# maxall41/RustSASA

Measured on AMD Instinct MI355X. Metric: structures/sec on AF2 E. coli proteome (100 pts, 1.4 A probe), higher is better.
Workload: dtype f32

## Files before the change

rustsasa_amd/csrc/context.cpp:

```cpp
#include "engine_internal.h"

namespace rsasa {

const char *tuning_env(const char *name)
{
    static const bool on = [] { const char *v = std::getenv("RSASA_TUNING"); return v && std::atoi(v) != 0; }();
    return on ? std::getenv(name) : nullptr;
}

void generate_sphere_points(size_t n, float *x, float *y, float *z)
{
    const float pi = 3.14159274101257324219f;
    const float angle_increment = (2.0f * pi) * 1.618034f;
    const float inv_n = 1.0f / (float)n;
    for (size_t i = 0; i < n; i++) {
        const float fi = (float)i;
        const float t = fi * inv_n;
        const float inclination = acosf(1.0f - 2.0f * t);
        const float azimuth = angle_increment * fi;
        const float si = sinf(inclination);
        x[i] = si * cosf(azimuth);
        y[i] = si * sinf(azimuth);
        z[i] = cosf(inclination);
    }
// ... 410 lines not shown
        RS_HIP(ctx, hs.h_segments.regrow((n_seg_all + n_seg_all / 2 + 64) * sizeof(Segment)));
    }
    Segment *h_segments = static_cast<Segment *>(hs.h_segments.p);
    write_segments(bt.structure_offsets_host, S, h_segments, reinterpret_cast<uint32_t *>(h_segments + n_seg));

    const bool has_id = bt.id != nullptr;
    if ((rc = W.reserve_grid(ctx, N, S, n_seg_all, ctx->cell_capacity, has_tail, has_id))) return rc;
    if ((rc = W.reserve_occlusion(ctx, lat, N, has_id, has_id, !bt.out_atom_sasa))) return rc;
    const bool keep_ids = W.keep_ids;
    if (keep_ids && pd.id32) return fail(ctx, RSASA_ERR_INTERNAL, "folded ids on a batch the per-atom kernels take");

    if (n_seg_all)
        RS_HIP(ctx, hipMemcpyAsync(W.segments.p, h_segments, n_seg_all * sizeof(Segment),
                                   hipMemcpyHostToDevice, st));

    BatchView v{};
    v.x = bt.x; v.y = bt.y; v.z = bt.z; v.radius = bt.radius; v.id = bt.id;
    v.id32 = pd.id32;
    v.ids_check = (has_id && !pd.ids_needed_known && !keep_ids && !tuning_env("RSASA_NO_ID_CHECK")) ? 1u : 0u;
    hs.ids_check = v.ids_check != 0u;
    v.large_sids = reinterpret_cast<const uint32_t *>((const Segment *)W.segments.p + n_seg);
    v.n_large = (uint32_t)n_large;
    v.ids_tables = ctx->ids_unordered_hint ? 1u : 0u;
    v.radius8 = pd.radius8;
    v.radius_table = pd.radius_table;
    v.residue_offsets = bt.residue_offsets;
    v.n_atoms = (uint32_t)N; v.n_structures = (uint32_t)S; v.n_residues = (uint32_t)R;
    v.n_segments = (uint32_t)n_seg;
    v.probe = pd.probe;
    v.atom_sasa = bt.out_atom_sasa;
    W.grid_view(v);
    W.occlusion_view(v);
    v.residue_sasa = (R && bt.residue_offsets) ? bt.out_residue_sasa : nullptr;
    v.neighbor_counts = bt.out_neighbor_counts;

    if (ctx->timing) RS_HIP(ctx, hipEventRecord(W.ev[0], st));
    launch_grid_prepare(v, st);
    rsasa_context::Workspace &other = ctx->ws[pd.ws ^ 1];
    const bool chain = other.occ_recorded && !tuning_env("RSASA_FREE_OVERLAP");
    const bool overlap = ctx->overlap_tail && has_tail;
    if (overlap && (rc = ensure_side_stream(ctx))) return rc;
    if (overlap) {
        launch_sort_lds(v, st);
        RS_HIP(ctx, hipEventRecord(ctx->ev_fork, st));
        RS_HIP(ctx, hipStreamWaitEvent(ctx->side_stream, ctx->ev_fork, 0));
        launch_sort_tail(v, ctx->side_stream);
// ... 176 lines not shown
    if (e == hipSuccess) e = new_stream(ctx, &ctx->stream.h, 2);
    for (int w = 0; w < rsasa_context::kInFlight; w++) {
        for (int i = 0; i < 5 && e == hipSuccess; i++) e = hipEventCreate(&ctx->ws[w].ev[i].h);
        if (e == hipSuccess) e = hipEventCreateWithFlags(&ctx->ws[w].ev_occ.h, hipEventDisableTiming);
    }
    if (e == hipSuccess) e = hipEventCreateWithFlags(&ctx->ev_fork.h, hipEventDisableTiming);
    if (e == hipSuccess) e = hipEventCreateWithFlags(&ctx->ev_join.h, hipEventDisableTiming);
    if (e == hipSuccess) e = hipEventCreateWithFlags(&ctx->ev_link.h, hipEventDisableTiming);
    for (int i = 0; i < rsasa_context::kSlots && e == hipSuccess; i++) e = hipEventCreateWithFlags(&ctx->ev_copy[i].h, hipEventDisableTiming);
    for (int i = 0; i < rsasa_context::kSlots && e == hipSuccess; i++) e = hipEventCreateWithFlags(&ctx->ev_d2h[i].h, hipEventDisableTiming);
    for (int i = 0; i < rsasa_context::kSlots && e == hipSuccess; i++) {
        e = ctx->slot[i].h_status.regrow(sizeof(BatchStatus));
        if (e == hipSuccess) std::memset(ctx->slot[i].h_status.p, 0, sizeof(BatchStatus));
        if (e == hipSuccess) e = hipEventCreateWithFlags(&ctx->ev_done[i].h, hipEventDisableTiming);
    }
    if (e != hipSuccess) {
        rsasa_context_destroy(ctx);
        return RSASA_ERR_HIP;
    }
    if (const char *v = tuning_env("RSASA_OCCLUSION_KERNEL")) ctx->tuning.kernel_version = std::atoi(v);
    if (const char *v = tuning_env("RSASA_ATOMS_PER_WAVE")) ctx->tuning.atoms_per_wave = (uint32_t)std::atoi(v);
    if (const char *v = tuning_env("RSASA_OVERLAP_TAIL")) ctx->overlap_tail = std::atoi(v) != 0;
    if (const char *v = tuning_env("RSASA_SMALL_PATH")) ctx->small_path = std::atoi(v) != 0;
    *out_ctx = ctx;
    return RSASA_OK;
}

extern "C" {

int rsasa_context_destroy(rsasa_context_t *ctx)
{
    if (!ctx) return RSASA_OK;
    if (HostStream *hs = ctx->host_stream) {
        {
            std::unique_lock<std::mutex> lk(hs->mu);
            hs->cv_done.wait(lk, [&] { for (auto &j : hs->jobs) if (!j->done) return false; return true; });
            hs->quit = true;
        }
        hs->cv_work.notify_all();
        for (auto &t : hs->th)
            if (t.joinable()) t.join();
        for (rsasa_context *sc : hs->sub) rsasa_context_destroy(sc);
        delete hs;
        ctx->host_stream = nullptr;
    }
    DeviceGuard guard(ctx->device);
// ... 253 lines not shown
```

rustsasa_amd/csrc/device_types.h:

```cpp
#pragma once
#include <hip/hip_runtime.h>
#include <stdint.h>

namespace rsasa {

struct StructGrid {
    float min_x, min_y, min_z;
    float inv_cell;
    uint32_t dim_x, dim_y, dim_z;
    uint32_t cell_base;
    float max_r;
    float cell_size;
    uint32_t n_cells;
    uint32_t atom_begin;
    uint32_t n_atoms;
    uint32_t sorted_base;
    uint32_t in_lds;
    uint32_t odd_radii;
};
static_assert(sizeof(StructGrid) == 64, "StructGrid layout");

struct StructAcc {
    int min_x, min_y, min_z;
    int max_x, max_y, max_z;
// ... 63 lines not shown
    StructGrid *grids;
    uint32_t *sid_sorted;
    uint32_t *cell_of, *rank_of;
    uint32_t *deferred_list;
    uint32_t *claim;
    uint32_t *ids_seg;
    uint32_t ids_seg_words;
    uint32_t *cells;
    uint64_t cell_capacity;
    uint4 *windows;
    uint32_t window_capacity;
    uint32_t *scan_block_sums;
    GridSums *grid_sums;
    float4 *sorted_xyzr;
    uint32_t *sorted_orig;
    uint64_t *sorted_id;
    uint32_t *sorted_id32;
    BatchStatus *status;
    float *atom_sasa;
    float *residue_sasa;
    uint32_t *neighbor_counts;
    uint32_t *defer_flag;
    float max_r_override = __builtin_nanf("");
};

struct NbInfo {
    unsigned long long total;
    unsigned long long max_k;
    unsigned long long spill_entries;
    unsigned long long spill_atoms;
    unsigned long long spill_cursor;
    unsigned long long spill_recs;
    unsigned long long mismatch;
    unsigned long long pad;
};
static_assert(sizeof(NbInfo) == 64, "NbInfo layout");
struct NbKey {
    unsigned long long key;
    float thr;
    uint32_t pad;
};
struct NbSpillRec {
    unsigned long long off, base;
    uint32_t k, pad;
};
struct NbArgs {
// ... 71 lines not shown
void launch_accessible_points(const PtArgs &a, hipStream_t stream);
void launch_contact_points(const CtArgs &c, hipStream_t stream);
void launch_neighbor_scan(const NbArgs &a, hipStream_t stream);
void launch_group_order(const GpArgs &g, hipStream_t stream);
void launch_group_points(const GpArgs &g, hipStream_t stream);
void launch_unpack_atoms(const void *records, uint32_t n_atoms, float *x, float *y, float *z, float *r, uint64_t *id,
                         const void *hdr_src, void *hdr_dst, uint32_t hdr_bytes, hipStream_t stream);
void launch_expand_frames(const float *xyz, const float *radius, const uint64_t *id,
                          const uint32_t *res_off, uint32_t n_atoms, uint32_t n_frames, uint32_t res_stride,
                          float *x, float *y, float *z, float *r, uint64_t *id_out,
                          uint32_t *res_out, hipStream_t stream);

constexpr uint32_t kSegmentAtoms = 4096;
constexpr uint32_t kScanBlocks = 1024;
constexpr uint32_t kWindowCells = 36864;
constexpr uint32_t kIdSlotsSmall = 8192, kIdAtomsSmall = 4096, kIdSlotsLarge = 73728, kIdAtomsLarge = 55296;
constexpr uint32_t kLdsMaxAtoms = 65536;

__host__ __device__ inline uint32_t grid_group_shift(uint32_t n_atoms, uint32_t n_cells)
{
    const float per_cell = (float)n_atoms / (float)(n_cells ? n_cells : 1u);
    return per_cell >= 1.0f ? 0u : per_cell >= 0.6f ? 1u : per_cell >= 0.3f ? 2u : 3u;
}
__host__ __device__ constexpr uint32_t lds_cell_slots(uint32_t n_cells) { return (n_cells + 1u + 7u) & ~7u; }
__host__ __device__ constexpr uint32_t grid_windows(uint32_t n_cells) { return (n_cells + kWindowCells - 1u) / kWindowCells; }

}
```

rustsasa_amd/csrc/device_utils.h:

```cpp
#pragma once
#include "device_types.h"

namespace rsasa {
namespace {

constexpr int kWave = 64;


__device__ __forceinline__ int f2ord(float f)
{
    int b = __float_as_int(f);
    return b >= 0 ? b : b ^ 0x7FFFFFFF;
}
__device__ __forceinline__ float ord2f(int o)
{
    return __int_as_float(o >= 0 ? o : o ^ 0x7FFFFFFF);
}

__device__ __forceinline__ uint32_t f2u_sat(float v)
{
    if (!(v > 0.0f)) return 0u;
    if (v >= 4294967296.0f) return 0xFFFFFFFFu;
    return (uint32_t)v;
}
// ... 30 lines not shown
__device__ __forceinline__ uint32_t block_incl_scan(uint32_t v, uint32_t *smem, uint32_t &total)
{
    static_assert(NW <= kWave, "one lane per wave");
    const uint32_t l = lane_id();
    const uint32_t w = (uint32_t)__builtin_amdgcn_readfirstlane((int)(threadIdx.x / kWave));
    const uint32_t inc = wave_incl_scan(v);
    __syncthreads();
    if (l == kWave - 1) smem[w] = inc;
    __syncthreads();
    const uint32_t s = l < (uint32_t)NW ? smem[l] : 0u;
    const uint32_t sc = wave_incl_scan(s);
    total = (uint32_t)__builtin_amdgcn_readlane((int)sc, kWave - 1);
    return inc + (uint32_t)__builtin_amdgcn_readlane((int)(sc - s), (int)w);
}

__device__ __forceinline__ bool batch_aborted(const BatchStatus *st)
{
    return (st->overflow | st->grid_too_large) != 0;
}

__device__ __forceinline__ void cell_coords(const StructGrid &g, float x, float y, float z,
                                            uint32_t &cx, uint32_t &cy, uint32_t &cz)
{
    cx = min(f2u_sat((x - g.min_x) * g.inv_cell), g.dim_x - 1u);
    cy = min(f2u_sat((y - g.min_y) * g.inv_cell), g.dim_y - 1u);
    cz = min(f2u_sat((z - g.min_z) * g.inv_cell), g.dim_z - 1u);
}


__device__ __forceinline__ uint32_t load_cell_start(const uint32_t *cells, uint32_t idx, bool rel16)
{
    return rel16 ? (uint32_t)reinterpret_cast<const uint16_t *>(cells)[idx] : cells[idx];
}

__device__ __forceinline__ void load_cell_start2(const uint32_t *cells, uint32_t idx0, uint32_t idx1, bool rel16,
                                                 uint32_t &v0, uint32_t &v1)
{
    if (rel16) {
        const uint16_t *c16 = reinterpret_cast<const uint16_t *>(cells);
        const uint16_t a = c16[idx0], b = c16[idx1];
        v0 = a;
        v1 = b;
    } else {
        const uint32_t a = cells[idx0], b = cells[idx1];
        v0 = a;
        v1 = b;
    }
// ... 19 lines not shown
```

rustsasa_amd/csrc/engine_internal.h:

```cpp
#pragma once
#include "../../include/rustsasa_amd.h"

#include <hip/hip_runtime.h>

#include <algorithm>
#include <chrono>
#include <atomic>
#include <cmath>
#include <cstdio>
#include <cstdlib>
#include <cstring>
#include <condition_variable>
#include <deque>
#include <map>
#include <memory>
#include <mutex>
#include <thread>
#include <new>
#include <string>
#include <utility>
#include <vector>

#include <pthread.h>
#include <sched.h>
// ... 264 lines not shown
    rsasa_context *sub[kMaxWorkers] = {};
    std::thread th[kMaxWorkers];
    std::mutex mu;
    std::condition_variable cv_work, cv_done;
    std::deque<std::shared_ptr<Job>> jobs;
    uint64_t next_ticket = 1;
    LinkGate gate;
    bool quit = false;
};

}

using namespace rsasa;

struct rsasa_context {
    int device = 0;
    NodeCpus node;
    Stream stream;
    std::recursive_mutex mu;
    std::string last_error;
    int simd_width = 8;
    bool timing = false;
    bool small_path = true;
    bool overlap_tail = false;
    Stream side_stream;
    Event ev_fork, ev_join;
    rsasa_timings_t timings{};
    bool timings_valid = false;

    struct Workspace {
        DeviceBuffer segments, acc, grids, grid_sums, sid_sorted, deferred_list, cell_of, rank_of, cells, windows, scan_sums,
            sorted_xyzr, sorted_orig, sorted_id, sorted_id32, status, atom_sasa, claim, ids_seg;
        Event ev[5];
        Event ev_occ;
        bool occ_recorded = false;
        uint64_t cell_capacity = 0;
        uint32_t window_capacity = 0, ids_seg_words = 0;
        bool has_id = false, keep_ids = false, id_bitmaps = false, own_atom_sasa = false;

        int reserve_sorted(rsasa_context *ctx, size_t N, size_t cell_words, bool has_id);
        void sorted_view(BatchView &v) const;
        int reserve_grid(rsasa_context *ctx, size_t N, size_t S, size_t n_seg_all, uint64_t &cell_capacity, bool has_tail, bool has_id);
        void grid_view(BatchView &v) const;
        int reserve_occlusion(rsasa_context *ctx, const Lattice &lat, size_t N, bool has_id, bool id_bitmaps, bool own_atom_sasa);
        void occlusion_view(BatchView &v) const;
    } ws[2];
// ... 188 lines not shown
```

rustsasa_amd/csrc/host_batch.cpp:

```cpp
#include "engine_internal.h"

namespace {

bool small_grid(const float mn_in[3], const float mx_in[3], float max_r, float probe, uint32_t n_atoms,
                StructGrid *out)
{
    const float cell = probe + max_r;
    const float inv = 1.0f / cell;
    if (!(cell > 0.0f) || !(inv < INFINITY) || !(cell < INFINITY)) return false;
    StructGrid g{};
    unsigned long long nc = 1;
    uint32_t d[3];
    const float mn[3] = {mn_in[0] - cell, mn_in[1] - cell, mn_in[2] - cell};
    const float mx[3] = {mx_in[0] + cell, mx_in[1] + cell, mx_in[2] + cell};
    for (int k = 0; k < 3; k++) {
        const float e = ceilf((mx[k] - mn[k]) * inv);
        if (!(e >= 0.0f) || e >= 2147483648.0f) return false;
        d[k] = (uint32_t)e + 1u;
        nc *= d[k];
        if (nc > 64ull * kWindowCells) return false;
    }
    g.min_x = mn[0]; g.min_y = mn[1]; g.min_z = mn[2];
    g.inv_cell = inv;
    g.dim_x = d[0]; g.dim_y = d[1]; g.dim_z = d[2];
// ... 11 lines not shown

}

namespace rsasa {

bool small_structure_grid(const SmallSource &src, uint32_t begin, uint32_t end, float probe, StructGrid *out)
{
    float mn[3] = {INFINITY, INFINITY, INFINITY}, mx[3] = {-INFINITY, -INFINITY, -INFINITY}, mr = 0.0f;
    bool finite = true, odd_r = false;
    for (uint32_t i = begin; i < end; i++) {
        float p[3], r;
        if (src.aos) { p[0] = src.aos[i].position[0]; p[1] = src.aos[i].position[1]; p[2] = src.aos[i].position[2]; r = src.aos[i].radius; }
        else { p[0] = src.x[i]; p[1] = src.y[i]; p[2] = src.z[i]; r = src.radius[i]; }
        for (int k = 0; k < 3; k++) {
            mn[k] = fminf(mn[k], p[k]);
            mx[k] = fmaxf(mx[k], p[k]);
            finite &= std::isfinite(p[k]);
        }
        mr = fmaxf(mr, r);
        finite &= std::isfinite(r);
        odd_r |= !(r >= 0.0f && r <= 64.0f) || !(fmaxf(fmaxf(fabsf(p[0]), fabsf(p[1])), fabsf(p[2])) <= 1e8f);
    }
    if (!finite || !small_grid(mn, mx, mr, probe, end - begin, out)) return false;
    out->odd_radii = (odd_r ? 1u : 0u) | (grid_group_shift(out->n_atoms, out->n_cells) << 8);
    return true;
}

void small_fill(const SmallSource &src, uint32_t begin, uint32_t end, const SmallLayout &lay, char *h, size_t at)
{
    const size_t n = end - begin;
    float *x = (float *)(h + lay.o_x) + at, *y = (float *)(h + lay.o_y) + at, *z = (float *)(h + lay.o_z) + at, *r = (float *)(h + lay.o_r) + at;
    uint64_t *id = lay.has_id ? (uint64_t *)(h + lay.o_id) + at : nullptr;
    if (src.aos) {
        const rsasa_atom_t *a = src.aos + begin;
        for (size_t i = 0; i < n; i++) {
            x[i] = a[i].position[0];
            y[i] = a[i].position[1];
            z[i] = a[i].position[2];
            r[i] = a[i].radius;
        }
        if (id)
            for (size_t i = 0; i < n; i++) id[i] = a[i].id;
        return;
    }
    std::memcpy(x, src.x + begin, n * 4);
    std::memcpy(y, src.y + begin, n * 4);
    std::memcpy(z, src.z + begin, n * 4);
// ... 1082 lines not shown
```

rustsasa_amd/csrc/kernels.hip:

```cpp
#include "device_utils.h"

#include <algorithm>

namespace rsasa {

namespace {


__global__ void k_init_acc(StructAcc *acc, uint32_t n_structures, BatchStatus *status, uint32_t ids_needed, uint32_t *ids_seg, uint32_t ids_seg_words)
{
    uint32_t s = blockIdx.x * blockDim.x + threadIdx.x;
    for (uint32_t i = s; ids_seg && i < 2u * ids_seg_words; i += gridDim.x * blockDim.x) ids_seg[i] = 0u;
    if (s == 0) {
        status->overflow = 0;
        status->grid_too_large = 0;
        status->bad_input = 0;
        status->deferred = 0;
        status->total_cells = 0;
        status->tail_cell_begin = 0;
        status->tail_atom_base = 0;
        status->n_windows = 0;
        status->grid_cells = 0;
        status->ids_needed = ids_needed;
        status->ids_unordered = 0;
// ... 143 lines not shown
    float mx[3] = {ord2f(a.max_x) + cell, ord2f(a.max_y) + cell, ord2f(a.max_z) + cell};
    uint32_t d[3];
#pragma unroll
    for (int k = 0; k < 3; k++)
        d[k] = f2u_sat(ceilf((mx[k] - mn[k]) * inv)) + 1u;
    unsigned long long nc = (unsigned long long)d[0] * d[1] * d[2];
    if (a.n_atoms == 0) {
        nc = 1; d[0] = d[1] = d[2] = 1;
        mn[0] = mn[1] = mn[2] = 0.0f;
        inv = 1.0f; cell = 1.0f;
    } else if (!(cell > 0.0f) || !(inv < __int_as_float(0x7F800000)) || !(cell < __int_as_float(0x7F800000))) {
        bad = true; nc = 1; d[0] = d[1] = d[2] = 1;
    }
    if (nc > 0x7FFFFFFFull || (a.n_atoms != 0 && (d[0] == 0u || d[1] == 0u || d[2] == 0u))) { too_large = true; nc = 1; d[0] = d[1] = d[2] = 1; }
    g.min_x = mn[0]; g.min_y = mn[1]; g.min_z = mn[2];
    g.inv_cell = inv;
    g.dim_x = d[0]; g.dim_y = d[1]; g.dim_z = d[2];
    g.max_r = max_r;
    g.cell_size = cell;
    g.n_cells = (uint32_t)nc;
    g.atom_begin = a.n_atoms ? a.first_atom : 0u;
    g.n_atoms = a.n_atoms;
    g.in_lds = a.n_atoms < kLdsMaxAtoms ? 1u : 0u;
    g.odd_radii = ((uint32_t)a.odd_radii & 7u) | (grid_group_shift(a.n_atoms, (uint32_t)nc) << 8);
    return g;
}

template <int NW>
__device__ __forceinline__ GridSums block_scan_sums(GridSums &v, unsigned long long (*part)[4])
{
    const uint32_t l = lane_id(), wv = threadIdx.x / kWave;
#pragma unroll
    for (int d = 1; d < kWave; d <<= 1) {
        const unsigned long long t0 = __shfl_up(v.cells_s, d, kWave), t1 = __shfl_up(v.cells_l, d, kWave);
        const unsigned long long t2 = __shfl_up(v.atoms_s, d, kWave), t3 = __shfl_up(v.atoms_l, d, kWave);
        if (l >= (uint32_t)d) { v.cells_s += t0; v.cells_l += t1; v.atoms_s += t2; v.atoms_l += t3; }
    }
    __syncthreads();
    if (l == kWave - 1) { part[wv][0] = v.cells_s; part[wv][1] = v.cells_l; part[wv][2] = v.atoms_s; part[wv][3] = v.atoms_l; }
    __syncthreads();
    unsigned long long off[4] = {0, 0, 0, 0}, tot[4] = {0, 0, 0, 0};
#pragma unroll
    for (int i = 0; i < NW; i++) {
#pragma unroll
        for (int k = 0; k < 4; k++) {
            const unsigned long long x = part[i][k];
            if ((uint32_t)i < wv) off[k] += x;
            tot[k] += x;
        }
    }
    v.cells_s += off[0]; v.cells_l += off[1]; v.atoms_s += off[2]; v.atoms_l += off[3];
    return GridSums{tot[0], tot[1], tot[2], tot[3]};
}

__global__ __launch_bounds__(256) void k_grid_params(BatchView b)
{
    __shared__ unsigned long long part[4][4];
    const uint32_t s = blockIdx.x * blockDim.x + threadIdx.x;
    GridSums v = {0, 0, 0, 0};
    unsigned long long n_cells = 0;
    if (s < b.n_structures) {
        bool bad = false, too_large = false;
        const StructGrid g = make_grid(b.acc[s], b.probe, b.max_r_override, bad, too_large);
        b.grids[s] = g;
        if (bad) b.status->bad_input = 1u;
        if (too_large) b.status->grid_too_large = 1u;
        if (g.in_lds) { v.cells_s = lds_cell_slots(g.n_cells); v.atoms_s = g.n_atoms | ((unsigned long long)grid_windows(g.n_cells) << 32); }
        else { v.cells_l = g.n_cells; v.atoms_l = g.n_atoms; }
        n_cells = g.n_cells;
    }
#pragma unroll
    for (int d = kWave / 2; d > 0; d >>= 1) n_cells += __shfl_xor(n_cells, d, kWave);
    if (lane_id() == 0 && n_cells) atomicAdd((unsigned long long *)&b.status->grid_cells, n_cells);
    const GridSums tot = block_scan_sums<4>(v, part);
    if (threadIdx.x == 0) b.grid_sums[blockIdx.x] = tot;
}

template <int NW>
__global__ __launch_bounds__(NW * kWave) void k_grid_scan(BatchView b, uint32_t n_parts)
{
    __shared__ unsigned long long part[NW][4];
    GridSums carry = {0, 0, 0, 0};
    for (uint32_t base = 0; base < n_parts; base += blockDim.x) {
        const uint32_t i = base + threadIdx.x;
        GridSums mine = {0, 0, 0, 0};
        if (i < n_parts) mine = b.grid_sums[i];
        GridSums v = mine;
        const GridSums tot = block_scan_sums<NW>(v, part);
        if (i < n_parts)
            b.grid_sums[i] = GridSums{carry.cells_s + v.cells_s - mine.cells_s, carry.cells_l + v.cells_l - mine.cells_l,
                                      carry.atoms_s + v.atoms_s - mine.atoms_s, carry.atoms_l + v.atoms_l - mine.atoms_l};
        carry.cells_s += tot.cells_s; carry.cells_l += tot.cells_l;
        carry.atoms_s += tot.atoms_s; carry.atoms_l += tot.atoms_l;
        __syncthreads();
    }
    if (threadIdx.x == 0) {
// ... 526 lines not shown
```

rustsasa_amd/csrc/neighbors.hip:

```cpp
#include "device_utils.h"

#include <algorithm>

namespace rsasa {
namespace {

constexpr uint32_t kNbStage = 512;
constexpr uint32_t kNbScanBlocks = 1024;

__device__ __forceinline__ uint32_t nb_runs(const BatchView &b, const StructGrid &g, const float4 me, uint32_t *s_excl,
                                            uint32_t *s_start)
{
    const uint32_t lane = lane_id();
    uint32_t cx, cy, cz;
    cell_coords(g, me.x, me.y, me.z, cx, cy, cz);
    uint32_t run_start = 0, run_len = 0;
    if (lane < 25) {
        const int yy = (int)cy + (int)(lane % 5u) - 2;
        const int zz = (int)cz + (int)(lane / 5u) - 2;
        if (yy >= 0 && yy < (int)g.dim_y && zz >= 0 && zz < (int)g.dim_z) {
            const uint32_t x0 = cx >= 2u ? cx - 2u : 0u;
            const uint32_t x1 = min(cx + 2u, g.dim_x - 1u);
            const uint32_t c0 = g.cell_base + x0 + (uint32_t)yy * g.dim_x + (uint32_t)zz * g.dim_x * g.dim_y;
            const bool rel16 = g.in_lds != 0u;
            const uint32_t first = load_cell_start(b.cells, c0, rel16);
            run_len = load_cell_start(b.cells, c0 + (x1 - x0) + 1u, rel16) - first;
            run_start = (rel16 ? g.sorted_base : 0u) + first;
        }
    }
    const uint32_t run_incl = wave_incl_scan(run_len);
    if (lane < 32) {
        s_excl[lane] = lane < 25 ? run_incl - run_len : 0xFFFFFFFFu;
        s_start[lane] = run_start;
    }
    wave_lds_fence();
    return wave_bcast(run_incl, 31);
}

__device__ __forceinline__ uint32_t nb_pos(const uint32_t *s_excl, const uint32_t *s_start, uint32_t f)
{
    uint32_t lo = 0;
#pragma unroll
    for (int step = 16; step > 0; step >>= 1)
        if (s_excl[lo + step] <= f) lo += step;
    return s_start[lo] + (f - s_excl[lo]);
// ... 304 lines not shown
```

rustsasa_amd/csrc/occlusion_fast.inc:

```

constexpr int kFastCap = 144;
constexpr uint32_t kFastMaxSwept = 256;
constexpr uint32_t kFastMaxRem = 4;
constexpr int kFastAtomsPerWave = 10;
constexpr int kTileSteps = 2;
constexpr int kCandPad = 8 * kTileSteps;


__device__ __forceinline__ float uniform_f(float v)
{
    return __int_as_float(__builtin_amdgcn_readfirstlane(__float_as_int(v)));
}

__device__ __forceinline__ void prologue_runs(const OccArgs3 &a, uint32_t first, uint32_t n_mine, float probe,
                                              float4 *scratch, uint2 (*runs)[25], float *srs)
{
    const uint32_t lane = lane_id();
    if (lane < n_mine) {
        const uint32_t pa = first + lane;
        const float4 m = a.sorted_xyzr[pa];
        const StructGrid g = a.grids[a.sid[pa]];
        const float tol = 8.0f * 1.1920929e-7f * (float)max(max(g.dim_x, g.dim_y), g.dim_z) + 1e-5f;
        const float sr = m.w + g.max_r + 2.0f * probe;
        const float fx = (m.x - g.min_x) * g.inv_cell;
        const float fy = (m.y - g.min_y) * g.inv_cell;
        const float fz = (m.z - g.min_z) * g.inv_cell;
        const int cx = (int)min((uint32_t)fmaxf(fx, 0.0f), g.dim_x - 1u);
        const int cy = (int)min((uint32_t)fmaxf(fy, 0.0f), g.dim_y - 1u);
        const int cz = (int)min((uint32_t)fmaxf(fz, 0.0f), g.dim_z - 1u);
        const float srn = sr * g.inv_cell;
        const uint32_t dim_xy = g.dim_x * g.dim_y;
        float4 *rec = scratch + 4u * lane;
        rec[0] = make_float4(fx, fy - (float)cy, fz - (float)cz, srn * srn * 1.00001f);
        rec[1] = make_float4(tol, __int_as_float(cx), __int_as_float(cy), __int_as_float(cz));
        rec[2] = make_float4(__uint_as_float(g.dim_x), __uint_as_float(g.dim_y), __uint_as_float(g.dim_z),
                             __uint_as_float(g.cell_base + (uint32_t)cy * g.dim_x + (uint32_t)cz * dim_xy));
        rec[3] = make_float4(__uint_as_float(dim_xy), __uint_as_float(g.in_lds ? g.sorted_base : 0xFFFFFFFFu), 0.f, 0.f);
        srs[lane] = sr;
    }
    wave_lds_fence();
    for (uint32_t idx = lane; idx < n_mine * 25u; idx += 64u) {
        const uint32_t at = (idx * 5243u) >> 17;
        const uint32_t r = idx - at * 25u;
        const int rdz = (int)((r * 13u) >> 6) - 2;
        const int rdy = (int)r - (rdz + 2) * 5 - 2;
        const float4 *rec = scratch + 4u * at;
        const float4 r0 = rec[0], r1 = rec[1], r2 = rec[2];
        const float fx = r0.x, uy = r0.y, uz = r0.z, thr = r0.w, tol = r1.x;
        const int cx = __float_as_int(r1.y), cy = __float_as_int(r1.z), cz = __float_as_int(r1.w);
        const uint32_t dim_x = __float_as_uint(r2.x), dim_y = __float_as_uint(r2.y), dim_z = __float_as_uint(r2.z);
        float gy = rdy > 0 ? (float)rdy - uy : (rdy < 0 ? uy - (float)(rdy + 1) : 0.0f);
        float gz = rdz > 0 ? (float)rdz - uz : (rdz < 0 ? uz - (float)(rdz + 1) : 0.0f);
        gy = fmaxf(gy - tol, 0.0f);
        gz = fmaxf(gz - tol, 0.0f);
        const float b2 = __builtin_fmaf(-gy, gy, __builtin_fmaf(-gz, gz, thr));
        const uint32_t yy = (uint32_t)(cy + rdy), zz = (uint32_t)(cz + rdz);
        uint32_t run_start = 0, run_len = 0;
        if (yy < dim_y && zz < dim_z && b2 >= 0.0f) {
            const float wx = __builtin_amdgcn_sqrtf(b2) * 1.0001f + tol;
            const int x0 = max(max((int)floorf(fx - wx), cx - 2), 0);
            const int x1 = min(min((int)floorf(fx + wx), cx + 2), (int)dim_x - 1);
            const float4 r3 = rec[3];
            const uint32_t dim_xy = __float_as_uint(r3.x), rel_base = __float_as_uint(r3.y);
            const bool rel16 = rel_base != 0xFFFFFFFFu;
            const uint32_t c0 = __float_as_uint(r2.w) + (uint32_t)(rdy * (int)dim_x) + (uint32_t)(rdz * (int)dim_xy) + (uint32_t)x0;
            const uint32_t first = load_cell_start(a.cells, c0, rel16);
            run_len = load_cell_start(a.cells, c0 + (uint32_t)(x1 - x0) + 1u, rel16) - first;
            run_start = (rel16 ? rel_base : 0u) + first;
        }
        runs[at][r] = make_uint2(run_start, run_len);
    }
    wave_lds_fence();
}

template <bool HAS_ID, bool HAS_REM, bool HALF1>
__global__ __launch_bounds__(256) void k_occlusion_fast(OccArgs3 a)
{
    if (batch_aborted(a.status)) return;
    __shared__ float4 s_cand[4][kFastCap + kCandPad];
    __shared__ int s_delta[4][32];
    __shared__ uint32_t s_mask[4][8];
    __shared__ uint32_t s_pts[4][64];
    __shared__ uint2 s_runs[4][kFastAtomsPerWave][25];
    __shared__ float s_sr[4][kFastAtomsPerWave];

    const float4 *__restrict__ sorted_xyzr = a.sorted_xyzr;
// ... 277 lines not shown
```

rustsasa_amd/csrc/occlusion_mx.inc:

```

#define MX_MIN_WAVES 7
constexpr int kMxCap = 128;
constexpr uint32_t kMxUnion = 256;
constexpr uint32_t kMxMinAtoms = 32768;
constexpr uint32_t kMxMaxPoints = 1344;
constexpr uint32_t kMxAtoms = 64;
constexpr uint32_t kMxAtomsMulti = 16;
#define MX_MAX_SGPR 96
constexpr float kMxNearScale2 = 1.8f;
constexpr uint32_t kMxXShift = 3;

typedef float mx_f4 __attribute__((ext_vector_type(4)));
typedef float mx_f16v __attribute__((ext_vector_type(16)));
typedef _Float16 mx_h4 __attribute__((ext_vector_type(4)));
typedef __fp16 mx_h2 __attribute__((ext_vector_type(2)));

__device__ __forceinline__ uint32_t pack_f16_rtz(float lo, float hi)
{
    return __builtin_bit_cast(uint32_t, __builtin_amdgcn_cvt_pkrtz(lo, hi));
}

__device__ __forceinline__ uint32_t max3u(uint32_t a, uint32_t b, uint32_t c) { return max(max(a, b), c); }

__device__ __forceinline__ bool is_negative_bits(uint32_t u) { return (u - 0x80000001u) <= 0x7F7FFFFFu; }
// ... 239 lines not shown
    uint32_t cxyz;
    {
        cxyz = (cx & 1023u) | ((cy & 1023u) << 10) | ((cz & 1023u) << 20);
        const uint32_t bx = cx >> my_shift;
        const uint32_t p_sid = (uint32_t)__builtin_amdgcn_update_dpp(0, (int)my_sid, 0x138, 0xf, 0xf, false);
        const uint32_t p_cy = (uint32_t)__builtin_amdgcn_update_dpp(0, (int)cy, 0x138, 0xf, 0xf, false);
        const uint32_t p_cz = (uint32_t)__builtin_amdgcn_update_dpp(0, (int)cz, 0x138, 0xf, 0xf, false);
        const uint32_t p_bx = (uint32_t)__builtin_amdgcn_update_dpp(0, (int)bx, 0x138, 0xf, 0xf, false);
        starts = ballot64(lane == 0u || p_sid != my_sid || p_cy != cy || p_cz != cz || p_bx != bx);
    }
    __builtin_amdgcn_s_setprio(0);
    wave_lds_fence();
    const unsigned long long mine_mask = n_mine >= 64u ? ~0ull : ((1ull << n_mine) - 1ull);

    constexpr uint32_t kDeferred = 0xFFFFFFFFu;
    uint32_t my_result = kDeferred;

    const mx_f4 zero4 = {0.f, 0.f, 0.f, 0.f};
    const mx_f16v zero16 = {0.f, 0.f, 0.f, 0.f, 0.f, 0.f, 0.f, 0.f, 0.f, 0.f, 0.f, 0.f, 0.f, 0.f, 0.f, 0.f};

    uint32_t g0 = 0;
    uint32_t cur_sid = 0xFFFFFFFFu;
    uint32_t dim_x = 1, dim_y = 1, dim_z = 1, cell_base = 0, rel_base = 0;
    bool rel16 = false;
    float max_r = 0.f;
    bool not_mine = false;
    while (g0 < n_mine) {
        uint32_t g1;
        {
            const unsigned long long later = starts & mine_mask & ~((2ull << g0) - 1ull);
            g1 = later ? (uint32_t)__builtin_ctzll(later) : n_mine;
        }
        const uint32_t sid_g = readlane_u(my_sid, g0);
        if (sid_g != cur_sid) {
            const StructGrid g = a.grids[sid_g];
            dim_x = (uint32_t)__builtin_amdgcn_readfirstlane((int)g.dim_x);
            dim_y = (uint32_t)__builtin_amdgcn_readfirstlane((int)g.dim_y);
            dim_z = (uint32_t)__builtin_amdgcn_readfirstlane((int)g.dim_z);
            cell_base = (uint32_t)__builtin_amdgcn_readfirstlane((int)g.cell_base);
            rel16 = __builtin_amdgcn_readfirstlane((int)g.in_lds) != 0;
            rel_base = rel16 ? (uint32_t)__builtin_amdgcn_readfirstlane((int)g.sorted_base) : 0u;
            max_r = uniform_f(g.max_r);
            not_mine = a.ids_check != 0u && (((uint32_t)__builtin_amdgcn_readfirstlane((int)g.odd_radii) >> 1) & 1u) != (HAS_ID ? 1u : 0u);
            cur_sid = sid_g;
        }
        if (not_mine) {
            if (kPersist && g0 == 0u && lane == 0u) s_blk[w][3] = s_blk[w][2] + next_claim;
            g0 = g1;
            continue;
        }
        const uint32_t gxyz = readlane_u(cxyz, g0);
        const uint32_t gcy = (gxyz >> 10) & 1023u, gcz = gxyz >> 20;
        const uint32_t cx_first = gxyz & 1023u;
        __builtin_amdgcn_s_setprio(kMxPrioGroup);
        uint32_t U, run_start, excl, n_chunk;
        for (;;) {
            const uint32_t cx_last = readlane_u(cxyz, g1 - 1u) & 1023u;
            const uint32_t x_lo = cx_first >= 2u ? cx_first - 2u : 0u;
            const uint32_t x_hi = min(cx_last + 2u, dim_x - 1u);
            const uint32_t yy = gcy + (uint32_t)rdy, zz = gcz + (uint32_t)rdz;
            uint32_t run_len = 0;
            run_start = 0;
            if (lane < 25u && yy < dim_y && zz < dim_z) {
                const uint32_t c0 = cell_base + (zz * dim_y + yy) * dim_x + x_lo;
                uint32_t first, behind;
                load_cell_start2(cells, c0, c0 + (x_hi - x_lo) + 1u, rel16, first, behind);
                run_len = behind - first;
                run_start = rel_base + first;
            }
            const uint32_t incl = scan_lanes32(run_len);
            U = readlane_u(incl, 31);
            excl = incl - run_len;
            if (U <= kUnion || cx_last == cx_first) {
                const bool run_ne = run_len > 0u;
                const unsigned long long ne_mask = ballot64(run_ne);
                if (lane < 2u * (uint32_t)NS) s_mask[w][lane] = 0u;
                if (run_ne) s_delta[w][mbcnt64(ne_mask)] = (int)run_start - (int)excl;
                wave_lds_fence();
                if (run_ne && excl != 0u && excl <= kUnion) atomicOr(&s_mask[w][(excl - 1u) >> 5], 1u << ((excl - 1u) & 31u));
                wave_lds_fence();
                break;
            }
            const uint32_t mid = (cx_first + cx_last) >> 1;
            const unsigned long long other = ballot64((cxyz & 1023u) > mid) & ~((1ull << g0) - 1ull) & mine_mask;
            g1 = (uint32_t)__builtin_ctzll(other);
        }
        n_chunk = (min(U, kUnion) + 63u) >> 6;
        const uint32_t self0 = w_begin + g0 - readlane_u(run_start, 0);

// ... 321 lines not shown
```

rustsasa_amd/csrc/occlusion_v0.inc:

```
constexpr int kCandCap = 192;
constexpr int kCandFlush = 128;


template <int NCH, bool HAS_ID>
__global__ __launch_bounds__(256) void k_occlusion_v0(OccArgs a)
{
    const BatchView &b = a.b;
    if (batch_aborted(b.status)) return;
    __shared__ float4 s_cand[4][kCandCap];
    __shared__ uint32_t s_run_excl[4][32];
    __shared__ uint32_t s_run_start[4][32];

    const uint32_t lane = lane_id();
    const uint32_t w = threadIdx.x / kWave;
    uint32_t bid = blockIdx.x;
    {
        const uint32_t per = a.n_blocks / 8u;
        if (bid < per * 8u) bid = (bid % 8u) * per + bid / 8u;
    }
    const uint32_t p = bid * 4u + w;
    if (p >= b.n_atoms) return;

    const float probe = b.probe;
    const float4 me = b.sorted_xyzr[p];
    const StructGrid g = b.grids[b.sid_sorted[p]];
    const float R = me.w + probe;
    const float R2 = R * R;
    const float twoR = 2.0f * R;
    const float sr = me.w + g.max_r + 2.0f * probe;
    const float sr2 = sr * sr;
    unsigned long long my_id = 0;
    if (HAS_ID) my_id = b.sorted_id[p];

    uint32_t cx, cy, cz;
    cell_coords(g, me.x, me.y, me.z, cx, cy, cz);
    uint32_t run_start = 0, run_len = 0;
    if (lane < 25) {
        const int yy = (int)cy + (int)(lane % 5u) - 2;
        const int zz = (int)cz + (int)(lane / 5u) - 2;
        if (yy >= 0 && yy < (int)g.dim_y && zz >= 0 && zz < (int)g.dim_z) {
            const uint32_t x0 = cx >= 2u ? cx - 2u : 0u;
            const uint32_t x1 = min(cx + 2u, g.dim_x - 1u);
            const uint32_t c0 = g.cell_base + x0 + (uint32_t)yy * g.dim_x +
                                (uint32_t)zz * g.dim_x * g.dim_y;
            const bool rel16 = g.in_lds != 0u;
            const uint32_t first = load_cell_start(b.cells, c0, rel16);
            run_len = load_cell_start(b.cells, c0 + (x1 - x0) + 1u, rel16) - first;
            run_start = (rel16 ? g.sorted_base : 0u) + first;
        }
    }
    const uint32_t run_incl = wave_incl_scan(run_len);
    const uint32_t total = wave_bcast(run_incl, 31);
    if (lane < 32) {
        s_run_excl[w][lane] = lane < 25 ? run_incl - run_len : 0xFFFFFFFFu;
        s_run_start[w][lane] = run_start;
    }
    wave_lds_fence();

    const uint32_t n_chunks = (a.lat.n_points + kWave - 1) / kWave;
    float accessible = 0.0f;
    uint32_t k_total = 0;

    for (uint32_t ch0 = 0; ch0 < n_chunks; ch0 += NCH) {
        float sx[NCH], sy[NCH], sz[NCH];
        unsigned long long occ[NCH], rem[NCH];
// ... 105 lines not shown
```

rustsasa_amd/csrc/occlusion_v3.inc:

```

template <int CTRL, int ROW_MASK = 0xf>
__device__ __forceinline__ uint32_t dpp_zero(uint32_t src)
{
    return (uint32_t)__builtin_amdgcn_update_dpp(0, (int)src, CTRL, ROW_MASK, 0xf, true);
}

__device__ __forceinline__ uint32_t scan_lanes32(uint32_t v)
{
    v += dpp_zero<0x111>(v);
    v += dpp_zero<0x112>(v);
    v += dpp_zero<0x114>(v);
    v += dpp_zero<0x118>(v);
    v += dpp_zero<0x142, 0xa>(v);
    return v;
}

constexpr bool kFlatSweep = true;
constexpr int kSegCap = 64;
constexpr int kSegLanes = 16;
constexpr int kSegShift = 4;
constexpr int kMaxAtomsPerWave = 8;
constexpr int kListCap = 192;
constexpr int kListFlush = kListCap - 64;
constexpr float kNearScale2 = 1.5625f;
// ... 98 lines not shown
    rem_shift = max(rem_shift, 2u);
    const uint32_t rem_pt = lane & ((1u << rem_shift) - 1u);
    const uint32_t rem_grp = lane >> rem_shift;
    const uint32_t rem_groups = 64u >> rem_shift;
    float4 rp = make_float4(0.f, 0.f, 0.f, 0.f);
    if (rem_pt < n_rem) rp = lat4[n_fused + rem_pt];
    const unsigned long long rem_low = n_rem ? ((1ull << n_rem) - 1ull) : 0ull;

    const uint32_t seg_sub = lane & (uint32_t)(kSegLanes - 1), seg_grp = lane >> kSegShift;
    const uint32_t dummy_slot = (uint32_t)kListCap + lane;

  for (;;) {
    const uint32_t p_end = min(p_begin + apw, n_work);
    {
        const uint32_t n_mine = p_end - p_begin;
        for (uint32_t idx = lane; idx < n_mine * 25u; idx += 64u) {
            const uint32_t at = (idx * 5243u) >> 17;
            const uint32_t r = idx - at * 25u;
            const int rdz = (int)((r * 13u) >> 6) - 2;
            const int rdy = (int)r - (rdz + 2) * 5 - 2;
            const uint32_t pa = list_mode ? work_list[p_begin + at] : p_begin + at;
            const float4 m = sorted_xyzr[pa];
            const StructGrid g = grids[sid[pa]];
            const float tol = 8.0f * 1.1920929e-7f * (float)max(max(g.dim_x, g.dim_y), g.dim_z) + 1e-5f;
            const float sr = m.w + g.max_r + 2.0f * probe;
            const float fx = (m.x - g.min_x) * g.inv_cell;
            const float fy = (m.y - g.min_y) * g.inv_cell;
            const float fz = (m.z - g.min_z) * g.inv_cell;
            const int cx = (int)min((uint32_t)fmaxf(fx, 0.0f), g.dim_x - 1u);
            const int cy = (int)min((uint32_t)fmaxf(fy, 0.0f), g.dim_y - 1u);
            const int cz = (int)min((uint32_t)fmaxf(fz, 0.0f), g.dim_z - 1u);
            const float srn = sr * g.inv_cell;
            const float thr = srn * srn * 1.00001f;
            const float uy = fy - (float)cy, uz = fz - (float)cz;
            float gy = rdy > 0 ? (float)rdy - uy : (rdy < 0 ? uy - (float)(rdy + 1) : 0.0f);
            float gz = rdz > 0 ? (float)rdz - uz : (rdz < 0 ? uz - (float)(rdz + 1) : 0.0f);
            gy = fmaxf(gy - tol, 0.0f);
            gz = fmaxf(gz - tol, 0.0f);
            const float b2 = __builtin_fmaf(-gy, gy, __builtin_fmaf(-gz, gz, thr));
            const uint32_t yy = (uint32_t)(cy + rdy), zz = (uint32_t)(cz + rdz);
            uint32_t run_start = 0, run_len = 0;
            if (yy < g.dim_y && zz < g.dim_z && b2 >= 0.0f) {
                const float wx = __builtin_amdgcn_sqrtf(b2) * 1.0001f + tol;
                const int x0 = max(max((int)floorf(fx - wx), cx - 2), 0);
                const int x1 = min(min((int)floorf(fx + wx), cx + 2), (int)g.dim_x - 1);
                const uint32_t c0 = g.cell_base + (uint32_t)x0 + yy * g.dim_x + zz * g.dim_x * g.dim_y;
                const bool rel16 = g.in_lds != 0u;
                const uint32_t first = load_cell_start(cells, c0, rel16);
                run_len = load_cell_start(cells, c0 + (uint32_t)(x1 - x0) + 1u, rel16) - first;
                run_start = (rel16 ? g.sorted_base : 0u) + first;
            }
            s_runs[w][at][r] = make_uint2(run_start, run_len);
            if (r == 0u) s_sr[w][at] = sr;
        }
        wave_lds_fence();
    }

    for (uint32_t pi = p_begin; pi < p_end; pi++) {
        const uint32_t at = pi - p_begin;
        const uint32_t p = list_mode ? work_list[pi] : pi;
        const float4 me = sorted_xyzr[p];
        const float R = me.w + probe;
        const float R2 = R * R;
        const float twoR = 2.0f * R;
        const float sr = s_sr[w][at];
        const float sr2 = sr * sr;
        const float near2 = kNearScale2 * R2;
        unsigned long long my_id = 0;
// ... 285 lines not shown
```

Measured before the change: 1.319 million.

## Merge pairs of x cells for sparse small grids to shrink cell tables

For sparse structures whose grid fits in LDS (group shift 3), the grid's x dimension is halved so each stored cell covers two logical x cells, with a flag bit in odd_radii. Cell coordinate, reach and run-range calculations in all occlusion and neighbor kernels are adjusted to map logical x ranges onto the wider cells. The goal is fewer cell-start entries to build, scan and store in LDS, and fewer run boundaries per lookup. The trade-off is that each run can hold more candidate atoms to test, and grid_cells accounting can optionally report stored cells instead of logical ones.

```diff
diff --git a/rustsasa_amd/csrc/context.cpp b/rustsasa_amd/csrc/context.cpp
--- a/rustsasa_amd/csrc/context.cpp
+++ b/rustsasa_amd/csrc/context.cpp
@@ -456,6 +456,7 @@
     v.large_sids = reinterpret_cast<const uint32_t *>((const Segment *)W.segments.p + n_seg);
     v.n_large = (uint32_t)n_large;
     v.ids_tables = ctx->ids_unordered_hint ? 1u : 0u;
+    v.count_stored = ctx->count_stored ? 1u : 0u;
     v.radius8 = pd.radius8;
     v.radius_table = pd.radius_table;
     v.residue_offsets = bt.residue_offsets;
@@ -678,6 +679,7 @@
     if (const char *v = tuning_env("RSASA_ATOMS_PER_WAVE")) ctx->tuning.atoms_per_wave = (uint32_t)std::atoi(v);
     if (const char *v = tuning_env("RSASA_OVERLAP_TAIL")) ctx->overlap_tail = std::atoi(v) != 0;
     if (const char *v = tuning_env("RSASA_SMALL_PATH")) ctx->small_path = std::atoi(v) != 0;
+    if (const char *v = tuning_env("RSASA_COUNT_STORED_CELLS")) ctx->count_stored = std::atoi(v) != 0;
     *out_ctx = ctx;
     return RSASA_OK;
 }
diff --git a/rustsasa_amd/csrc/device_types.h b/rustsasa_amd/csrc/device_types.h
--- a/rustsasa_amd/csrc/device_types.h
+++ b/rustsasa_amd/csrc/device_types.h
@@ -109,6 +109,7 @@
     uint32_t *neighbor_counts;
     uint32_t *defer_flag;
     float max_r_override = __builtin_nanf("");
+    uint32_t count_stored = 0;
 };
 
 struct NbInfo {
@@ -226,6 +227,21 @@
     const float per_cell = (float)n_atoms / (float)(n_cells ? n_cells : 1u);
     return per_cell >= 1.0f ? 0u : per_cell >= 0.6f ? 1u : per_cell >= 0.3f ? 2u : 3u;
 }
+constexpr uint32_t kGridWideX = 1u << 10;
+__host__ __device__ inline void grid_choose_x_cells(StructGrid &g, uint32_t flags)
+{
+    uint32_t shift = grid_group_shift(g.n_atoms, g.n_cells);
+    uint32_t wide = 0u;
+    if (shift == 3u && g.in_lds) {
+        wide = kGridWideX;
+        shift = 2u;
+        g.dim_x = (g.dim_x + 1u) >> 1;
+        g.n_cells = g.dim_x * g.dim_y * g.dim_z;
+    }
+    g.odd_radii = flags | (shift << 8) | wide;
+}
+__host__ __device__ inline uint32_t grid_x_wide(const StructGrid &g) { return (g.odd_radii >> 10) & 1u; }
+__host__ __device__ inline uint32_t grid_x_reach(const StructGrid &g) { return 2u - grid_x_wide(g); }
 __host__ __device__ constexpr uint32_t lds_cell_slots(uint32_t n_cells) { return (n_cells + 1u + 7u) & ~7u; }
 __host__ __device__ constexpr uint32_t grid_windows(uint32_t n_cells) { return (n_cells + kWindowCells - 1u) / kWindowCells; }
 
diff --git a/rustsasa_amd/csrc/device_utils.h b/rustsasa_amd/csrc/device_utils.h
--- a/rustsasa_amd/csrc/device_utils.h
+++ b/rustsasa_amd/csrc/device_utils.h
@@ -76,7 +76,7 @@
 __device__ __forceinline__ void cell_coords(const StructGrid &g, float x, float y, float z,
                                             uint32_t &cx, uint32_t &cy, uint32_t &cz)
 {
-    cx = min(f2u_sat((x - g.min_x) * g.inv_cell), g.dim_x - 1u);
+    cx = min(f2u_sat((x - g.min_x) * g.inv_cell) >> grid_x_wide(g), g.dim_x - 1u);
     cy = min(f2u_sat((y - g.min_y) * g.inv_cell), g.dim_y - 1u);
     cz = min(f2u_sat((z - g.min_z) * g.inv_cell), g.dim_z - 1u);
 }
diff --git a/rustsasa_amd/csrc/engine_internal.h b/rustsasa_amd/csrc/engine_internal.h
--- a/rustsasa_amd/csrc/engine_internal.h
+++ b/rustsasa_amd/csrc/engine_internal.h
@@ -310,6 +310,7 @@
     int simd_width = 8;
     bool timing = false;
     bool small_path = true;
+    bool count_stored = false;
     bool overlap_tail = false;
     Stream side_stream;
     Event ev_fork, ev_join;
diff --git a/rustsasa_amd/csrc/host_batch.cpp b/rustsasa_amd/csrc/host_batch.cpp
--- a/rustsasa_amd/csrc/host_batch.cpp
+++ b/rustsasa_amd/csrc/host_batch.cpp
@@ -57,7 +57,7 @@
         odd_r |= !(r >= 0.0f && r <= 64.0f) || !(fmaxf(fmaxf(fabsf(p[0]), fabsf(p[1])), fabsf(p[2])) <= 1e8f);
     }
     if (!finite || !small_grid(mn, mx, mr, probe, end - begin, out)) return false;
-    out->odd_radii = (odd_r ? 1u : 0u) | (grid_group_shift(out->n_atoms, out->n_cells) << 8);
+    grid_choose_x_cells(*out, odd_r ? 1u : 0u);
     return true;
 }
 
diff --git a/rustsasa_amd/csrc/kernels.hip b/rustsasa_amd/csrc/kernels.hip
--- a/rustsasa_amd/csrc/kernels.hip
+++ b/rustsasa_amd/csrc/kernels.hip
@@ -189,7 +189,7 @@
     g.atom_begin = a.n_atoms ? a.first_atom : 0u;
     g.n_atoms = a.n_atoms;
     g.in_lds = a.n_atoms < kLdsMaxAtoms ? 1u : 0u;
-    g.odd_radii = ((uint32_t)a.odd_radii & 7u) | (grid_group_shift(a.n_atoms, (uint32_t)nc) << 8);
+    g.odd_radii = (uint32_t)a.odd_radii & 7u;
     return g;
 }
 
@@ -225,20 +225,22 @@
     __shared__ unsigned long long part[4][4];
     const uint32_t s = blockIdx.x * blockDim.x + threadIdx.x;
     GridSums v = {0, 0, 0, 0};
-    unsigned long long n_cells = 0;
+    unsigned long long n_cells = 0, n_stored = 0;
     if (s < b.n_structures) {
         bool bad = false, too_large = false;
-        const StructGrid g = make_grid(b.acc[s], b.probe, b.max_r_override, bad, too_large);
+        StructGrid g = make_grid(b.acc[s], b.probe, b.max_r_override, bad, too_large);
+        n_cells = g.n_cells;
+        grid_choose_x_cells(g, g.odd_radii);
+        n_stored = g.n_cells;
         b.grids[s] = g;
         if (bad) b.status->bad_input = 1u;
         if (too_large) b.status->grid_too_large = 1u;
         if (g.in_lds) { v.cells_s = lds_cell_slots(g.n_cells); v.atoms_s = g.n_atoms | ((unsigned long long)grid_windows(g.n_cells) << 32); }
         else { v.cells_l = g.n_cells; v.atoms_l = g.n_atoms; }
-        n_cells = g.n_cells;
-    }
-#pragma unroll
-    for (int d = kWave / 2; d > 0; d >>= 1) n_cells += __shfl_xor(n_cells, d, kWave);
-    if (lane_id() == 0 && n_cells) atomicAdd((unsigned long long *)&b.status->grid_cells, n_cells);
+    }
+#pragma unroll
+    for (int d = kWave / 2; d > 0; d >>= 1) { n_cells += __shfl_xor(n_cells, d, kWave); n_stored += __shfl_xor(n_stored, d, kWave); }
+    if (lane_id() == 0 && n_cells) atomicAdd((unsigned long long *)&b.status->grid_cells, b.count_stored ? n_stored : n_cells);
     const GridSums tot = block_scan_sums<4>(v, part);
     if (threadIdx.x == 0) b.grid_sums[blockIdx.x] = tot;
 }
diff --git a/rustsasa_amd/csrc/neighbors.hip b/rustsasa_amd/csrc/neighbors.hip
--- a/rustsasa_amd/csrc/neighbors.hip
+++ b/rustsasa_amd/csrc/neighbors.hip
@@ -19,8 +19,9 @@
         const int yy = (int)cy + (int)(lane % 5u) - 2;
         const int zz = (int)cz + (int)(lane / 5u) - 2;
         if (yy >= 0 && yy < (int)g.dim_y && zz >= 0 && zz < (int)g.dim_z) {
-            const uint32_t x0 = cx >= 2u ? cx - 2u : 0u;
-            const uint32_t x1 = min(cx + 2u, g.dim_x - 1u);
+            const uint32_t reach = grid_x_reach(g);
+            const uint32_t x0 = cx >= reach ? cx - reach : 0u;
+            const uint32_t x1 = min(cx + reach, g.dim_x - 1u);
             const uint32_t c0 = g.cell_base + x0 + (uint32_t)yy * g.dim_x + (uint32_t)zz * g.dim_x * g.dim_y;
             const bool rel16 = g.in_lds != 0u;
             const uint32_t first = load_cell_start(b.cells, c0, rel16);
diff --git a/rustsasa_amd/csrc/occlusion_fast.inc b/rustsasa_amd/csrc/occlusion_fast.inc
--- a/rustsasa_amd/csrc/occlusion_fast.inc
+++ b/rustsasa_amd/csrc/occlusion_fast.inc
@@ -20,12 +20,13 @@
         const uint32_t pa = first + lane;
         const float4 m = a.sorted_xyzr[pa];
         const StructGrid g = a.grids[a.sid[pa]];
-        const float tol = 8.0f * 1.1920929e-7f * (float)max(max(g.dim_x, g.dim_y), g.dim_z) + 1e-5f;
+        const uint32_t xw = grid_x_wide(g), dim_xn = g.dim_x << xw;
+        const float tol = 8.0f * 1.1920929e-7f * (float)max(max(dim_xn, g.dim_y), g.dim_z) + 1e-5f;
         const float sr = m.w + g.max_r + 2.0f * probe;
         const float fx = (m.x - g.min_x) * g.inv_cell;
         const float fy = (m.y - g.min_y) * g.inv_cell;
         const float fz = (m.z - g.min_z) * g.inv_cell;
-        const int cx = (int)min((uint32_t)fmaxf(fx, 0.0f), g.dim_x - 1u);
+        const int cx = (int)min((uint32_t)fmaxf(fx, 0.0f), dim_xn - 1u);
         const int cy = (int)min((uint32_t)fmaxf(fy, 0.0f), g.dim_y - 1u);
         const int cz = (int)min((uint32_t)fmaxf(fz, 0.0f), g.dim_z - 1u);
         const float srn = sr * g.inv_cell;
@@ -35,7 +36,8 @@
         rec[1] = make_float4(tol, __int_as_float(cx), __int_as_float(cy), __int_as_float(cz));
         rec[2] = make_float4(__uint_as_float(g.dim_x), __uint_as_float(g.dim_y), __uint_as_float(g.dim_z),
                              __uint_as_float(g.cell_base + (uint32_t)cy * g.dim_x + (uint32_t)cz * dim_xy));
-        rec[3] = make_float4(__uint_as_float(dim_xy), __uint_as_float(g.in_lds ? g.sorted_base : 0xFFFFFFFFu), 0.f, 0.f);
+        rec[3] = make_float4(__uint_as_float(dim_xy), __uint_as_float(g.in_lds ? g.sorted_base : 0xFFFFFFFFu),
+                             __uint_as_float(xw), 0.f);
         srs[lane] = sr;
     }
     wave_lds_fence();
@@ -58,10 +60,10 @@
         uint32_t run_start = 0, run_len = 0;
         if (yy < dim_y && zz < dim_z && b2 >= 0.0f) {
             const float wx = __builtin_amdgcn_sqrtf(b2) * 1.0001f + tol;
-            const int x0 = max(max((int)floorf(fx - wx), cx - 2), 0);
-            const int x1 = min(min((int)floorf(fx + wx), cx + 2), (int)dim_x - 1);
             const float4 r3 = rec[3];
-            const uint32_t dim_xy = __float_as_uint(r3.x), rel_base = __float_as_uint(r3.y);
+            const uint32_t dim_xy = __float_as_uint(r3.x), rel_base = __float_as_uint(r3.y), xw = __float_as_uint(r3.z);
+            const int x0 = max(max((int)floorf(fx - wx), cx - 2), 0) >> xw;
+            const int x1 = max(min(min((int)floorf(fx + wx), cx + 2) >> xw, (int)dim_x - 1), x0);
             const bool rel16 = rel_base != 0xFFFFFFFFu;
             const uint32_t c0 = __float_as_uint(r2.w) + (uint32_t)(rdy * (int)dim_x) + (uint32_t)(rdz * (int)dim_xy) + (uint32_t)x0;
             const uint32_t first = load_cell_start(a.cells, c0, rel16);
diff --git a/rustsasa_amd/csrc/occlusion_mx.inc b/rustsasa_amd/csrc/occlusion_mx.inc
--- a/rustsasa_amd/csrc/occlusion_mx.inc
+++ b/rustsasa_amd/csrc/occlusion_mx.inc
@@ -285,7 +285,7 @@
     uint32_t g0 = 0;
     uint32_t cur_sid = 0xFFFFFFFFu;
     uint32_t dim_x = 1, dim_y = 1, dim_z = 1, cell_base = 0, rel_base = 0;
-    bool rel16 = false;
+    uint32_t cell_kind = 0;
     float max_r = 0.f;
     bool not_mine = false;
     while (g0 < n_mine) {
@@ -301,8 +301,8 @@
             dim_y = (uint32_t)__builtin_amdgcn_readfirstlane((int)g.dim_y);
             dim_z = (uint32_t)__builtin_amdgcn_readfirstlane((int)g.dim_z);
             cell_base = (uint32_t)__builtin_amdgcn_readfirstlane((int)g.cell_base);
-            rel16 = __builtin_amdgcn_readfirstlane((int)g.in_lds) != 0;
-            rel_base = rel16 ? (uint32_t)__builtin_amdgcn_readfirstlane((int)g.sorted_base) : 0u;
+            cell_kind = (uint32_t)__builtin_amdgcn_readfirstlane((int)((g.in_lds != 0u ? 1u : 0u) | (grid_x_wide(g) << 1)));
+            rel_base = (cell_kind & 1u) ? (uint32_t)__builtin_amdgcn_readfirstlane((int)g.sorted_base) : 0u;
             max_r = uniform_f(g.max_r);
             not_mine = a.ids_check != 0u && (((uint32_t)__builtin_amdgcn_readfirstlane((int)g.odd_radii) >> 1) & 1u) != (HAS_ID ? 1u : 0u);
             cur_sid = sid_g;
@@ -319,15 +319,16 @@
         uint32_t U, run_start, excl, n_chunk;
         for (;;) {
             const uint32_t cx_last = readlane_u(cxyz, g1 - 1u) & 1023u;
-            const uint32_t x_lo = cx_first >= 2u ? cx_first - 2u : 0u;
-            const uint32_t x_hi = min(cx_last + 2u, dim_x - 1u);
+            const uint32_t reach = 2u - (cell_kind >> 1);
+            const uint32_t x_lo = cx_first >= reach ? cx_first - reach : 0u;
+            const uint32_t x_hi = min(cx_last + reach, dim_x - 1u);
             const uint32_t yy = gcy + (uint32_t)rdy, zz = gcz + (uint32_t)rdz;
             uint32_t run_len = 0;
             run_start = 0;
             if (lane < 25u && yy < dim_y && zz < dim_z) {
                 const uint32_t c0 = cell_base + (zz * dim_y + yy) * dim_x + x_lo;
                 uint32_t first, behind;
-                load_cell_start2(cells, c0, c0 + (x_hi - x_lo) + 1u, rel16, first, behind);
+                load_cell_start2(cells, c0, c0 + (x_hi - x_lo) + 1u, (cell_kind & 1u) != 0u, first, behind);
                 run_len = behind - first;
                 run_start = rel_base + first;
             }
diff --git a/rustsasa_amd/csrc/occlusion_v0.inc b/rustsasa_amd/csrc/occlusion_v0.inc
--- a/rustsasa_amd/csrc/occlusion_v0.inc
+++ b/rustsasa_amd/csrc/occlusion_v0.inc
@@ -39,8 +39,9 @@
         const int yy = (int)cy + (int)(lane % 5u) - 2;
         const int zz = (int)cz + (int)(lane / 5u) - 2;
         if (yy >= 0 && yy < (int)g.dim_y && zz >= 0 && zz < (int)g.dim_z) {
-            const uint32_t x0 = cx >= 2u ? cx - 2u : 0u;
-            const uint32_t x1 = min(cx + 2u, g.dim_x - 1u);
+            const uint32_t reach = grid_x_reach(g);
+            const uint32_t x0 = cx >= reach ? cx - reach : 0u;
+            const uint32_t x1 = min(cx + reach, g.dim_x - 1u);
             const uint32_t c0 = g.cell_base + x0 + (uint32_t)yy * g.dim_x +
                                 (uint32_t)zz * g.dim_x * g.dim_y;
             const bool rel16 = g.in_lds != 0u;
diff --git a/rustsasa_amd/csrc/occlusion_v3.inc b/rustsasa_amd/csrc/occlusion_v3.inc
--- a/rustsasa_amd/csrc/occlusion_v3.inc
+++ b/rustsasa_amd/csrc/occlusion_v3.inc
@@ -144,12 +144,13 @@
             const uint32_t pa = list_mode ? work_list[p_begin + at] : p_begin + at;
             const float4 m = sorted_xyzr[pa];
             const StructGrid g = grids[sid[pa]];
-            const float tol = 8.0f * 1.1920929e-7f * (float)max(max(g.dim_x, g.dim_y), g.dim_z) + 1e-5f;
+            const uint32_t xw = grid_x_wide(g), dim_xn = g.dim_x << xw;
+            const float tol = 8.0f * 1.1920929e-7f * (float)max(max(dim_xn, g.dim_y), g.dim_z) + 1e-5f;
             const float sr = m.w + g.max_r + 2.0f * probe;
             const float fx = (m.x - g.min_x) * g.inv_cell;
             const float fy = (m.y - g.min_y) * g.inv_cell;
             const float fz = (m.z - g.min_z) * g.inv_cell;
-            const int cx = (int)min((uint32_t)fmaxf(fx, 0.0f), g.dim_x - 1u);
+            const int cx = (int)min((uint32_t)fmaxf(fx, 0.0f), dim_xn - 1u);
             const int cy = (int)min((uint32_t)fmaxf(fy, 0.0f), g.dim_y - 1u);
             const int cz = (int)min((uint32_t)fmaxf(fz, 0.0f), g.dim_z - 1u);
             const float srn = sr * g.inv_cell;
@@ -164,8 +165,8 @@
             uint32_t run_start = 0, run_len = 0;
             if (yy < g.dim_y && zz < g.dim_z && b2 >= 0.0f) {
                 const float wx = __builtin_amdgcn_sqrtf(b2) * 1.0001f + tol;
-                const int x0 = max(max((int)floorf(fx - wx), cx - 2), 0);
-                const int x1 = min(min((int)floorf(fx + wx), cx + 2), (int)g.dim_x - 1);
+                const int x0 = max(max((int)floorf(fx - wx), cx - 2), 0) >> xw;
+                const int x1 = max(min(min((int)floorf(fx + wx), cx + 2) >> xw, (int)g.dim_x - 1), x0);
                 const uint32_t c0 = g.cell_base + (uint32_t)x0 + yy * g.dim_x + zz * g.dim_x * g.dim_y;
                 const bool rel16 = g.in_lds != 0u;
                 const uint32_t first = load_cell_start(cells, c0, rel16);
```

After: 1.342 million, median of 6. 1.02x the previous value.
